# RishWijewardhena/vision-textile-inspection

Hardware: AMD Instinct MI355X
Metric: frames/sec whole-node, YOLOv8n-seg 640x640 bs=64; mask IoU vs CPU ref (higher is better)
Workload: dtype f16x2

## Files before the change

vision-textile-inspection_amd/csrc/post.hip:

```cpp
#include <algorithm>
#include <cmath>
#include <cstdio>
#include <cstring>
#include <type_traits>
#include <vector>

#include "vti_internal.h"

namespace vti {

typedef _Float16 half_t;
typedef _Float16 half8 __attribute__((ext_vector_type(8)));
typedef float f32x4 __attribute__((ext_vector_type(4)));

struct LinTap { int s0, s1, a0, a1; };

__device__ __forceinline__ LinTap lin_tap(int d, int ssize, double scale, bool horizontal) {
    float f = (float)(((double)d + 0.5) * scale - 0.5);
    int s = (int)floorf(f);
    f -= (float)s;
    LinTap t;
    if (horizontal) {
        if (s < 0) { s = 0; f = 0.f; }
        if (s >= ssize - 1) { s = ssize - 1; f = 0.f; }
// ... 89 lines not shown
                    const int rr = i / (ncol * 3), j = i - rr * ncol * 3;
                    band[((size_t)rr * W + xb) * 3 + j] = s_px[rr][j];
                }
            }
        }
        return;
    }
    const bool src4 = ((uintptr_t)src & 3) == 0, out4 = ((uintptr_t)out & 3) == 0;
    const bool wide = src4 && (copy ? ((W0 | left) & 3) == 0 : (left & 1) == 0);
    for (int g = tid; g < (W >> 2); g += 256) {
        const int dx0 = 4 * g - left;
        const bool inside = dx0 >= 0 && dx0 + 3 < new_w;
        uint8_t* o = band + (size_t)g * 12;
        for (int rr = 0; rr < rows; ++rr, o += (size_t)W * 3) {
            const int dy = y0 + rr - top;
            unsigned w[3] = {0x72727272u, 0x72727272u, 0x72727272u};
            if (dy >= 0 && dy < new_h && dx0 + 3 >= 0 && dx0 < new_w) {
                if (copy) {
                    const uint8_t* s = src + ((long long)dy * W0 + dx0) * 3;
                    if (wide && inside) {
                        const unsigned* q = (const unsigned*)s;
                        w[0] = q[0]; w[1] = q[1]; w[2] = q[2];
                    } else {
#pragma unroll
                        for (int i = 0; i < 12; ++i) {
                            const int dx = dx0 + i / 3;
                            const unsigned v = dx >= 0 && dx < new_w ? s[i] : 114u;
                            w[i >> 2] = (w[i >> 2] & ~(255u << ((i & 3) * 8))) | (v << ((i & 3) * 8));
                        }
                    }
                } else {
                    const uint8_t* s0 = src + ((long long)(2 * dy) * W0 + 2 * dx0) * 3;
                    const uint8_t* s1 = s0 + (size_t)W0 * 3;
                    if (wide && inside) {
                        unsigned q0[6], q1[6];
#pragma unroll
                        for (int i = 0; i < 6; ++i) { q0[i] = ((const unsigned*)s0)[i]; q1[i] = ((const unsigned*)s1)[i]; }
#pragma unroll
                        for (int i = 0; i < 12; ++i) {
                            const int j = 6 * (i / 3) + i % 3;
                            const unsigned v = (lb_byte(q0, j) + lb_byte(q0, j + 3) + lb_byte(q1, j) + lb_byte(q1, j + 3) + 2) >> 2;
                            w[i >> 2] = (w[i >> 2] & ~(255u << ((i & 3) * 8))) | (v << ((i & 3) * 8));
                        }
                    } else {
#pragma unroll
                        for (int i = 0; i < 12; ++i) {
                            const int dx = dx0 + i / 3, j = 6 * (i / 3) + i % 3;
                            unsigned v = 114u;
                            if (dx >= 0 && dx < new_w) v = (s0[j] + s0[j + 3] + s1[j] + s1[j + 3] + 2) >> 2;
                            w[i >> 2] = (w[i >> 2] & ~(255u << ((i & 3) * 8))) | (v << ((i & 3) * 8));
                        }
                    }
                }
            }
            if (out4) {
                *(uint3*)o = make_uint3(w[0], w[1], w[2]);
            } else {
#pragma unroll
                for (int i = 0; i < 12; ++i) o[i] = (uint8_t)lb_byte(w, i);
            }
        }
    }
}

hipError_t launch_letterbox(const uint8_t* frames, int B, int H0, int W0, const FrameRow* table, uint8_t* out, int H, int W,
                            hipStream_t st) {
    if (B == 0) return hipSuccess;
    if (W & 3) return hipErrorInvalidValue;
    const dim3 grid((H + LB_ROWS - 1) / LB_ROWS, B);
    FrameRow one = {};
    if (table) hipLaunchKernelGGL(letterbox_rows_kernel<true>, grid, dim3(256), 0, st, frames, one, table, out, H, W);
    else {
        frame_row_fill(H, W, H0, W0, 0, one);
        hipLaunchKernelGGL(letterbox_rows_kernel<false>, grid, dim3(256), 0, st, frames, one, table, out, H, W);
    }
    return hipGetLastError();
}

constexpr int NMS_THREADS = 1024;
constexpr int NMS_LDS_BOX = 2048;
constexpr int NMS_LDS_KEYS = 2048;
constexpr float NMS_MAX_WH = 7680.0f;
constexpr int NMS_MAX_NMS = 30000;

static inline size_t nms_pow2(size_t n) { size_t p = 1; while (p < n) p <<= 1; return p; }
static inline size_t align256(size_t n) { return (n + 255) & ~(size_t)255; }

struct NmsWsLayout { size_t keys, keys2, boxes, area, cls, keep, kid, kcls, per_frame; };
static NmsWsLayout nms_layout(int A) {
    NmsWsLayout l;
    size_t off = 0;
    l.keys = off; off += align256(nms_pow2((size_t)A) * 8);
    l.keys2 = off; off += align256(nms_pow2((size_t)A) * 8);
    l.boxes = off; off += align256((size_t)A * 16);
    l.area = off; off += align256((size_t)A * 4);
    l.cls = off; off += align256((size_t)A * 4);
    l.keep = off; off += align256((size_t)A * 4);
    l.kid = off; off += align256((size_t)A * 4);
    l.kcls = off; off += align256((size_t)A * 4);
    l.per_frame = off;
    return l;
}
size_t nms_workspace_bytes(int B, int A) { return nms_layout(A).per_frame * (size_t)B + align256((size_t)B * 4) + align256((size_t)B * A * 8); }
float* nms_workspace_best(void* ws, int B, int A) { return (float*)((char*)ws + nms_layout(A).per_frame * (size_t)B + align256((size_t)B * 4)); }

__global__ __launch_bounds__(256) void nms_scan_kernel(const float* __restrict__ pred, int A, int nc, int nm, float conf,
                                                       char* ws, NmsWsLayout L, int* __restrict__ ncand, float* __restrict__ best_out) {
    const int b = blockIdx.y;
    const int no = 4 + nc + nm;
    float best;
    int j = 0;
    int a;
    if (((no | nc) & 3) == 0) {
        a = blockIdx.x * 64 + (threadIdx.x >> 2);
        const int q = threadIdx.x & 3;
        best = -INFINITY; j = 0x7fffffff;
        if (a < A) {
            const float4* row = (const float4*)(pred + ((size_t)b * A + a) * no + 4);
            constexpr int MAXV = 8;
            float4 v[MAXV];
#pragma unroll
            for (int u = 0; u < MAXV; ++u) {
                const int i = q + 4 * u;
                v[u] = row[i < (nc >> 2) ? i : 0];
            }
#pragma unroll
            for (int u = 0; u < MAXV; ++u) {
                const int i = q + 4 * u;
                if (i >= (nc >> 2)) continue;
                if (v[u].x > best) { best = v[u].x; j = 4 * i; }
                if (v[u].y > best) { best = v[u].y; j = 4 * i + 1; }
                if (v[u].z > best) { best = v[u].z; j = 4 * i + 2; }
                if (v[u].w > best) { best = v[u].w; j = 4 * i + 3; }
            }
            for (int i = q + 4 * MAXV; i < (nc >> 2); i += 4) {
                const float4 w = row[i];
                if (w.x > best) { best = w.x; j = 4 * i; }
                if (w.y > best) { best = w.y; j = 4 * i + 1; }
                if (w.z > best) { best = w.z; j = 4 * i + 2; }
                if (w.w > best) { best = w.w; j = 4 * i + 3; }
            }
        }
#pragma unroll
        for (int o = 1; o <= 2; o <<= 1) {
            const float ob = __shfl_xor(best, o);
            const int oj = __shfl_xor(j, o);
            if (ob > best || (ob == best && oj < j)) { best = ob; j = oj; }
        }
        if (q != 0 || a >= A) return;
    } else {
        a = blockIdx.x * 256 + threadIdx.x;
        if (a >= A) return;
        const float* P = pred + ((size_t)b * A + a) * no;
        best = P[4];
        for (int c = 1; c < nc; ++c) {
            const float v = P[4 + c];
            if (v > best) { best = v; j = c; }
        }
    }
    if (best_out) {
        *(float2*)(best_out + ((size_t)b * A + a) * 2) = make_float2(best, (float)(j == 0x7fffffff ? 0 : j));
        return;
    }
    if (best > conf) {
        char* wsb = ws + (size_t)b * L.per_frame;
        const int idx = atomicAdd(&ncand[b], 1);
        ((unsigned long long*)(wsb + L.keys))[idx] = ((unsigned long long)(~__float_as_uint(best)) << 32) | (unsigned)a;
        ((int*)(wsb + L.cls))[a] = j;
    }
}

#ifdef VTI_STAMPS
__device__ unsigned long long g_nms_stamps[4096 * 8];
#define NMS_STAMP(i)                                                                                   \
    do {                                                                                               \
        if (tid == 0 && b < 4096) {                                                                    \
            unsigned long long t_;                                                                     \
            asm volatile("s_memtime %0\n\ts_waitcnt lgkmcnt(0)" : "=s"(t_)::"memory");                 \
            g_nms_stamps[b * 8 + (i)] = t_;                                                            \
        }                                                                                              \
    } while (0)
#else
#define NMS_STAMP(i) do { } while (0)
#endif

template <typename KeyP, typename BoxP, typename FltP, typename IntP>
__device__ __forceinline__ void nms_body(const float* __restrict__ P, int A, int nc, int nm, int n, double iou, int max_det,
                                         int agnostic, float* __restrict__ D, int* __restrict__ counts, int b,
                                         const unsigned long long* __restrict__ g_keys_in, KeyP keys, BoxP boxes, FltP area,
                                         IntP keep, IntP kid, IntP kcls, unsigned char* suppressed,
                                         const int* __restrict__ cls_of) {
    const int tid = threadIdx.x;
    int Pn = 1;
    while (Pn < n) Pn <<= 1;
    for (int i = tid; i < Pn; i += NMS_THREADS) keys[i] = i < n ? g_keys_in[i] : ~0ull;
    __syncthreads();
    for (int k = 2; k <= Pn; k <<= 1) {
        for (int j = k >> 1; j > 0; j >>= 1) {
            for (int i = tid; i < Pn; i += NMS_THREADS) {
                const int ixj = i ^ j;
                if (ixj > i) {
                    const unsigned long long x = keys[i], y = keys[ixj];
                    const bool up = (i & k) == 0;
                    if ((x > y) == up) { keys[i] = y; keys[ixj] = x; }
                }
            }
            __syncthreads();
        }
    }
    NMS_STAMP(1);
    if (n > NMS_MAX_NMS) n = NMS_MAX_NMS;
    for (int i = tid; i < n; i += NMS_THREADS) {
        const int a = (int)(keys[i] & 0xffffffffu);
        const float* Pa = P + (size_t)a * (4 + nc + nm);
        const float cx = Pa[0], cy = Pa[1], w = Pa[2], h = Pa[3];
        const float dw = w / 2.0f, dh = h / 2.0f;
        const float off = agnostic ? 0.0f : (float)cls_of[a] * NMS_MAX_WH;
        f32x4 bx;
        bx[0] = (cx - dw) + off; bx[1] = (cy - dh) + off; bx[2] = (cx + dw) + off; bx[3] = (cy + dh) + off;
        boxes[i] = bx;
        area[i] = (bx[2] - bx[0]) * (bx[3] - bx[1]);
        suppressed[i] = 0;
    }
    __syncthreads();
    NMS_STAMP(2);
    __shared__ unsigned long long s_rows[64];
    __shared__ int s_kept;
    auto iou_gt = [&](const f32x4& bi, float ai, const f32x4& bj, float aj) -> bool {
        const float xx1 = fmaxf(bi[0], bj[0]), yy1 = fmaxf(bi[1], bj[1]);
        const float xx2 = fminf(bi[2], bj[2]), yy2 = fminf(bi[3], bj[3]);
        const float w = fmaxf(0.0f, xx2 - xx1), h = fmaxf(0.0f, yy2 - yy1);
        const float inter = w * h;
        const float ovr = inter / (ai + aj - inter);
        return (double)ovr > iou;
    };
    int kept = 0;
    if (tid == 0) s_kept = 0;
    for (int base = 0; base < n && kept < max_det; base += 64) {
        const int cnt = min(64, n - base);
        if (tid < 64) s_rows[tid] = 0;
        __syncthreads();
        for (int e = tid; e < 64 * 16; e += NMS_THREADS) {
            const int i = e >> 4, jg = (e & 15) * 4;
            if (i >= cnt || jg + 3 <= i) continue;
            const f32x4 bi = boxes[base + i];
            const float ai = area[base + i];
            unsigned long long m = 0;
            f32x4 bj4[4];
            float aj4[4];
#pragma unroll
            for (int k = 0; k < 4; ++k) {
                const int jc = jg + k < cnt ? jg + k : cnt - 1;
                bj4[k] = boxes[base + jc]; aj4[k] = area[base + jc];
            }
#pragma unroll
            for (int k = 0; k < 4; ++k) {
                const int j = jg + k;
                if (j > i && j < cnt && iou_gt(bi, ai, bj4[k], aj4[k])) m |= 1ull << j;
            }
            if (m) atomicOr(&s_rows[i], m);
        }
        __syncthreads();
        if (tid < 64) {
            const bool alive_l = tid < cnt && !suppressed[base + tid];
            unsigned long long alive = __ballot(alive_l);
            int k_ = kept;
            const unsigned long long myrow = s_rows[tid];
            const int row_lo = (int)(unsigned)myrow, row_hi = (int)(unsigned)(myrow >> 32);
            while (alive && k_ < max_det) {
                const int i = __ffsll((long long)alive) - 1;
                if (tid == 0) keep[k_] = base + i;
                ++k_;
                const unsigned long long ri = (unsigned long long)(unsigned)__builtin_amdgcn_readlane(row_lo, i) |
                                              ((unsigned long long)(unsigned)__builtin_amdgcn_readlane(row_hi, i) << 32);
                alive &= ~(ri | (1ull << i));
            }
            if (tid == 0) s_kept = k_;
        }
        __syncthreads();
        const int kept0 = kept;
        kept = s_kept;
        if (kept < max_det) {
            const int nk = kept - kept0;
            const int rest = n - (base + 64);
            int parts = 1;
            while (parts < 8 && rest * parts * 2 <= NMS_THREADS) parts <<= 1;
            const int part = tid & (parts - 1), lane_j = tid / parts, jstep = NMS_THREADS / parts;
            for (int j = base + 64 + lane_j; j < n; j += jstep) {
                if (suppressed[j]) continue;
                const f32x4 bj = boxes[j];
                const float aj = area[j];
                bool sup = false;
                for (int t = 4 * part; t < nk && !sup; t += 4 * parts) {
                    int ii[4];
                    f32x4 bk[4];
                    float ak[4];
#pragma unroll
                    for (int u = 0; u < 4; ++u) ii[u] = keep[kept0 + (t + u < nk ? t + u : nk - 1)];
#pragma unroll
                    for (int u = 0; u < 4; ++u) { bk[u] = boxes[ii[u]]; ak[u] = area[ii[u]]; }
#pragma unroll
                    for (int u = 0; u < 4; ++u) sup = sup | iou_gt(bk[u], ak[u], bj, aj);
                }
                if (sup) suppressed[j] = 1;
            }
        }
        __syncthreads();
    }
    NMS_STAMP(3);
    for (int k = tid; k < kept; k += NMS_THREADS) {
        const int a = (int)(keys[keep[k]] & 0xffffffffu);
        kid[k] = a;
        kcls[k] = cls_of[a];
    }
    __syncthreads();
    const int row = 6 + nm;
    const unsigned row_magic = (unsigned)((0x100000000ull + (unsigned)row - 1) / (unsigned)row);
    const int nel = kept * row, ntot = max_det * row;
    const int no_ = 4 + nc + nm;
    constexpr int OU = 8;
    for (int e0 = tid; e0 < nel; e0 += OU * NMS_THREADS) {
        float x1[OU], x2[OU];
        int fj[OU];
#pragma unroll
        for (int u = 0; u < OU; ++u) {
            const int e = e0 + u * NMS_THREADS;
            const int ec = e < nel ? e : 0;
            const int k = (int)__umulhi((unsigned)ec, row_magic), f = ec - k * row;
            const int a = kid[k], j = kcls[k];
            const int off1 = f < 4 ? (f & 1) : f == 4 ? 4 + j : f == 5 ? 0 : 4 + nc + (f - 6);
            const int off2 = f < 4 ? 2 + (f & 1) : off1;
            const float* Pa = P + (size_t)a * no_;
            x1[u] = Pa[off1]; x2[u] = Pa[off2];
            fj[u] = (f << 16) | j;
        }
#pragma unroll
        for (int u = 0; u < OU; ++u) {
            const int e = e0 + u * NMS_THREADS;
            const int f = fj[u] >> 16, j = fj[u] & 0xffff;
            const float d_ = x2[u] / 2.0f;
            const float v = f < 2 ? x1[u] - d_ : f < 4 ? x1[u] + d_ : f == 5 ? (float)j : x1[u];
            if (e < nel) D[e] = v;
        }
    }
    for (int e = nel + tid; e < ntot; e += NMS_THREADS) D[e] = 0.f;
    __syncthreads();
    NMS_STAMP(4);
    if (tid == 0) counts[b] = kept;
}

__global__ __launch_bounds__(NMS_THREADS) void nms_kernel(const float* __restrict__ pred, int A, int nc, int nm,
                                                          float conf, double iou, int max_det, int agnostic,
                                                          float* __restrict__ dets, int* __restrict__ counts,
                                                          char* ws, NmsWsLayout L, int* __restrict__ ncand,
                                                          const float* __restrict__ best) {
    extern __shared__ __attribute__((aligned(16))) char smem[];
    unsigned long long* lds_keys = (unsigned long long*)smem;
    f32x4* lds_boxes = (f32x4*)(smem + NMS_LDS_KEYS * 8);
    float* lds_area = (float*)(lds_boxes + NMS_LDS_BOX);
    int* lds_keep = (int*)(lds_area + NMS_LDS_BOX);
    unsigned char* suppressed = (unsigned char*)(lds_keep + 3 * NMS_LDS_BOX);

    const int b = blockIdx.x, tid = threadIdx.x;
    const int no = 4 + nc + nm;
    const float* P = pred + (size_t)b * no * A;
    char* wsb = ws + (size_t)b * L.per_frame;
    unsigned long long* g_keys = (unsigned long long*)(wsb + L.keys);
    const int* cls_of = (const int*)(wsb + L.cls);
    float* D = dets + (size_t)b * max_det * (6 + nm);
    __shared__ int s_cnt;
    if (best) {
        if (tid == 0) s_cnt = 0;
        __syncthreads();
        const float2* bp = (const float2*)best + (size_t)b * A;
        int* cls_w = (int*)(wsb + L.cls);
        for (int a0 = 0; a0 < A; a0 += 4 * NMS_THREADS) {
            float2 v[4];
#pragma unroll
            for (int u = 0; u < 4; ++u) { const int a = a0 + tid + u * NMS_THREADS; v[u] = bp[a < A ? a : A - 1]; }
#pragma unroll
            for (int u = 0; u < 4; ++u) {
                const int a = a0 + tid + u * NMS_THREADS;
                if (a < A && v[u].x > conf) {
                    const int idx = atomicAdd(&s_cnt, 1);
                    g_keys[idx] = ((unsigned long long)(~__float_as_uint(v[u].x)) << 32) | (unsigned)a;
                    cls_w[a] = (int)v[u].y;
                }
            }
        }
        __syncthreads();
        if (tid == 0) ncand[b] = s_cnt;
    }
    const int n = best ? s_cnt : ncand[b];
    if (n == 0) {
        if (tid == 0) counts[b] = 0;
        for (int i = tid; i < max_det * (6 + nm); i += NMS_THREADS) D[i] = 0.f;
        return;
    }
    NMS_STAMP(0);
    if (n <= NMS_LDS_BOX && max_det <= NMS_LDS_BOX) {
        nms_body(P, A, nc, nm, n, iou, max_det, agnostic, D, counts, b, g_keys, lds_keys, lds_boxes, lds_area, lds_keep,
                 lds_keep + NMS_LDS_BOX, lds_keep + 2 * NMS_LDS_BOX, suppressed, cls_of);
    } else {
        int* g_int = (int*)(wsb + L.keep);
        nms_body(P, A, nc, nm, n, iou, max_det, agnostic, D, counts, b, g_keys, (unsigned long long*)(wsb + L.keys2),
                 (f32x4*)(wsb + L.boxes), (float*)(wsb + L.area), g_int, (int*)(wsb + L.kid), (int*)(wsb + L.kcls), suppressed,
                 cls_of);
    }
}

hipError_t launch_anchor_best(const float* pred, int B, int A, int nc, int nm, float* best, hipStream_t st) {
    if (B == 0) return hipSuccess;
    const int apb = (((4 + nc + nm) | nc) & 3) == 0 ? 64 : 256;
    hipLaunchKernelGGL(nms_scan_kernel, dim3((A + apb - 1) / apb, B), dim3(256), 0, st, pred, A, nc, nm, 0.0f, (char*)nullptr, nms_layout(A),
                       (int*)nullptr, best);
    return hipGetLastError();
}

hipError_t launch_nms(const float* pred, const float* best, int B, int A, int nc, int nm, float conf, double iou, int max_det,
                      int agnostic, float* dets, int* counts, void* ws, hipStream_t st) {
    if (B == 0) return hipSuccess;
    const size_t lds = (size_t)NMS_LDS_KEYS * 8 + (size_t)NMS_LDS_BOX * 32 + (((size_t)A + 15) & ~(size_t)15);
    if (lds > 150 * 1024) return hipErrorInvalidValue;
    const NmsWsLayout L = nms_layout(A);
    int* ncand = (int*)((char*)ws + L.per_frame * (size_t)B);
    if (!best) {
        hipError_t e = hipMemsetAsync(ncand, 0, sizeof(int) * (size_t)B, st);
        if (e != hipSuccess) return e;
        const int apb = (((4 + nc + nm) | nc) & 3) == 0 ? 64 : 256;
        hipLaunchKernelGGL(nms_scan_kernel, dim3((A + apb - 1) / apb, B), dim3(256), 0, st, pred, A, nc, nm, conf, (char*)ws, L, ncand, (float*)nullptr);
    }
    const hipError_t e = launch_lds<nms_kernel>(dim3(B), dim3(NMS_THREADS), lds, st, pred, A, nc, nm, conf, iou, max_det, agnostic,
                                                dets, counts, (char*)ws, L, ncand, best);
#ifdef VTI_STAMPS
    {
        (void)hipStreamSynchronize(st);
        static int calls = 0;
        if (++calls == 3) {
            std::vector<unsigned long long> h(4096 * 8);
            std::vector<int> hc(B), hn(B);
            (void)hipMemcpyFromSymbol(h.data(), HIP_SYMBOL(g_nms_stamps), h.size() * 8);
            (void)hipMemcpy(hc.data(), counts, B * 4, hipMemcpyDeviceToHost);
            (void)hipMemcpy(hn.data(), ncand, B * 4, hipMemcpyDeviceToHost);
            const char* nm_[4] = {"sort", "boxes", "greedy", "output"};
            int worst = 0;
            for (int b = 1; b < B; ++b) if (h[b * 8 + 4] - h[b * 8] > h[worst * 8 + 4] - h[worst * 8]) worst = b;
            fprintf(stderr, "[nms stamps] slowest frame %d: candidates %d kept %d\n", worst, hn[worst], hc[worst]);
            for (int i = 0; i < 4; ++i) {
                std::vector<long long> d;
                for (int b = 0; b < B; ++b) if (hn[b] > 0) d.push_back((long long)(h[b * 8 + i + 1] - h[b * 8 + i]));
                std::sort(d.begin(), d.end());
                fprintf(stderr, "[nms stamps] %-7s median %8lld  max %8lld  slowest-frame %8lld cycles\n", nm_[i],
                        d.empty() ? 0 : d[d.size() / 2], d.empty() ? 0 : d.back(), (long long)(h[worst * 8 + i + 1] - h[worst * 8 + i]));
            }
        }
    }
#endif
    return e;
}

constexpr int MT = 64;
constexpr int ML = MT / 4 + 3;

__global__ __launch_bounds__(256) void mask_offsets_kernel(const int* __restrict__ counts, int B, int max_det,
                                                           int* __restrict__ offsets, int* __restrict__ nitems) {
    extern __shared__ int s_off[];
    for (int b = threadIdx.x; b < B; b += 256) {
        int c = counts[b];
        s_off[b + 1] = c < 0 ? 0 : (c > max_det ? max_det : c);
    }
    if (threadIdx.x == 0) { s_off[0] = 0; *nitems = 0; }
    __syncthreads();
    if (threadIdx.x == 0)
        for (int b = 0; b < B; ++b) s_off[b + 1] += s_off[b];
    __syncthreads();
    for (int b = threadIdx.x; b <= B; b += 256) offsets[b] = s_off[b];
}

__device__ __forceinline__ void mask_slot_owner(const int* __restrict__ offsets, int B, int slot, int& b, int& inst) {
    int lo = 0, hi = B;
    while (hi - lo > 1) { const int mid = (lo + hi) >> 1; if (offsets[mid] <= slot) lo = mid; else hi = mid; }
    b = lo; inst = slot - offsets[lo];
}
__device__ __forceinline__ bool mask_tile_rect(const float* __restrict__ d, int H, int W, int& tx0, int& tx1, int& ty0, int& ty1) {
    const int tiles_x = (W + MT - 1) / MT, tiles_y = (H + MT - 1) / MT;
    const float x1 = d[0] - 8.f, y1 = d[1] - 8.f, x2 = d[2] + 8.f, y2 = d[3] + 8.f;
    tx0 = (int)floorf(x1 / MT); tx1 = (int)floorf(x2 / MT); ty0 = (int)floorf(y1 / MT); ty1 = (int)floorf(y2 / MT);
    tx0 = max(tx0, 0); ty0 = max(ty0, 0); tx1 = min(tx1, tiles_x - 1); ty1 = min(ty1, tiles_y - 1);
    return tx1 >= tx0 && ty1 >= ty0;
}

template <bool FUSED_OFFSETS>
__global__ __launch_bounds__(256) void mask_clear_kernel(const int* __restrict__ counts, int* __restrict__ offsets, int* __restrict__ nitems,
                                                         int B, int max_det, int slot_bytes, int capacity, uint8_t* __restrict__ masks) {
    const int slot = blockIdx.x;
    int total;
    if constexpr (FUSED_OFFSETS) {
        __shared__ int s_c[1025];
        __shared__ int s_tot;
        if (threadIdx.x == 0) s_tot = 0;
        __syncthreads();
        int part = 0;
        for (int b = threadIdx.x; b < B; b += 256) {
            const int c = counts[b], cc = c < 0 ? 0 : (c > max_det ? max_det : c);
            part += cc;
            if (slot == 0) s_c[b + 1] = cc;
        }
        for (int o = 32; o > 0; o >>= 1) part += __shfl_xor(part, o);
        if ((threadIdx.x & 63) == 0) atomicAdd(&s_tot, part);
        __syncthreads();
        total = s_tot;
        if (slot == 0) {
            if (threadIdx.x == 0) {
                s_c[0] = 0; *nitems = 0;
                for (int b = 0; b < B; ++b) s_c[b + 1] += s_c[b];
            }
// ... 141 lines not shown

        const float thr = mode == VTI_MASK_SIGMOID ? 0.5f : 0.0f;
        const int wv = tid >> 6, ln = tid & 63;
        const int yw = __builtin_amdgcn_readfirstlane(y0 + 16 * wv);
        if (yw >= H) continue;
        const int xg = x0 + ln;
        int k0 = xg >= 2 ? (xg - 2) >> 2 : 0;
        k0 = k0 < Wp - 1 ? k0 : Wp - 1;
        const int k1 = k0 + (k0 < Wp - 1 ? 1 : 0);
        const float lx1 = xg >= 2 ? 0.125f + 0.25f * (float)((xg - 2) & 3) : 0.0f;
        const int rb = (yw >> 2) - 1;
        int ro[6];
#pragma unroll
        for (int j = 0; j < 6; ++j) {
            int rr = rb + j;
            rr = rr < 0 ? 0 : (rr > Hp - 1 ? Hp - 1 : rr);
            ro[j] = (rr - ly0) * (ML + 1);
        }
        const int valid = W - x0;
        const unsigned long long cmask = valid >= 64 ? ~0ull : ((1ull << valid) - 1ull);
        unsigned lo = 0u, hi = 0u;
        if (packing == VTI_PACK_U8) mask_rows16<true>(&low[0][0], ro, k0 - lx0, k1 - lx0, lx1, yw == 0, thr, lo, hi, masks + (size_t)slot * H * W, W, H, yw, xg);
        else mask_rows16<false>(&low[0][0], ro, k0 - lx0, k1 - lx0, lx1, yw == 0, thr, lo, hi, nullptr, W, H, yw, xg);
        lo &= (unsigned)cmask; hi &= (unsigned)(cmask >> 32);
        if (packing != VTI_PACK_U8 && ln < 16 && yw + ln < H) {
            const int wb = W >> 3;
            unsigned* o = (unsigned*)(masks + ((size_t)slot * H + yw + ln) * wb + (x0 >> 3));
            o[0] = lo;
            if (valid >= 64) o[1] = hi;
        }
    }
}

constexpr int MLP = ML + 2;
__device__ __forceinline__ void mask_tile_rows64(const float* lrow, float wy, bool first, float thr, unsigned& lo, unsigned& hi) {
    float vv[18];
#pragma unroll
    for (int j = 0; j < 18; ++j) {
        const float a = lrow[j], b = lrow[j + MLP];
        vv[j] = __builtin_fmaf(b - a, wy, a);
    }
    unsigned w[2] = {0u, 0u};
    if (thr == 0.0f) {
#pragma unroll
        for (int j = 0; j < 18; ++j) vv[j] = -vv[j];
#pragma unroll
        for (int hf = 0; hf < 2; ++hf) {
#pragma unroll
            for (int k = 31; k >= 0; --k) {
                const int px = 32 * hf + k;
                const int jj = ((px - 2) >> 2) + 1;
                const float wx = 0.125f + 0.25f * (float)((px + 2) & 3);
                float u = __builtin_fmaf(vv[jj + 1] - vv[jj], wx, vv[jj]);
                if (px < 2) u = first ? vv[1] + 0.0f : u;
                w[hf] = __builtin_amdgcn_alignbit(w[hf], __builtin_bit_cast(unsigned, u), 31);
            }
        }
    } else {
#pragma unroll
        for (int hf = 0; hf < 2; ++hf) {
#pragma unroll
            for (int k = 31; k >= 0; --k) {
                const int px = 32 * hf + k;
                const int jj = ((px - 2) >> 2) + 1;
                const float wx = 0.125f + 0.25f * (float)((px + 2) & 3);
                float v = __builtin_fmaf(vv[jj + 1] - vv[jj], wx, vv[jj]);
                if (px < 2) v = first ? vv[1] : v;
                asm("v_cmp_gt_f32 vcc, %1, %2\n\tv_addc_co_u32 %0, vcc, %0, %0, vcc" : "+v"(w[hf]) : "v"(v), "v"(thr) : "vcc");
            }
        }
    }
    lo = w[0]; hi = w[1];
}

#ifdef VTI_STAMPS
__device__ unsigned long long g_mask_acc[8];
#define MASK_T(i) do { unsigned long long t_; asm volatile("s_memtime %0\n\ts_waitcnt lgkmcnt(0)" : "=s"(t_)::"memory"); \
                       macc[i] += t_ - mprev; mprev = t_; } while (0)
#else
#define MASK_T(i) do { } while (0)
#endif

constexpr int MG = 16;
constexpr int MPTS = ML * ML;
constexpr int MTILES = (MPTS + 15) / 16;
constexpr int MJ = (MTILES + 3) / 4;
constexpr int MROUND = 64;

template <bool F16>
__device__ __forceinline__ float mask_coef_operands(const float (&cf)[32], uint4* dst) {
    float scale = 1.0f;
    if constexpr (F16) {
        float mx = 0.f;
#pragma unroll
        for (int k = 0; k < 32; ++k) mx = fmaxf(mx, fabsf(cf[k]));
        float inv = 1.0f;
        if (!(mx < 3.0e4f)) {
            const int e = (int)((__builtin_bit_cast(unsigned, mx) >> 23) & 255u) - 127 - 13;
            const int ec = e < -100 ? -100 : (e > 100 ? 100 : e);
            scale = __builtin_bit_cast(float, (unsigned)(ec + 127) << 23);
            inv = __builtin_bit_cast(float, (unsigned)(127 - ec) << 23);
        }
#pragma unroll
        for (int q = 0; q < 4; ++q) {
            half8 hh, hl;
#pragma unroll
            for (int k = 0; k < 8; ++k) {
                const float c = cf[8 * q + k] * inv;
                const half_t h = (half_t)c;
                hh[k] = h;
                hl[k] = (half_t)(c - (float)h);
            }
            dst[q] = __builtin_bit_cast(uint4, hh);
            dst[4 + q] = __builtin_bit_cast(uint4, hl);
        }
    } else {
#pragma unroll
        for (int q = 0; q < 8; ++q)
            dst[q] = __builtin_bit_cast(uint4, (f32x4){cf[4 * q], cf[4 * q + 1], cf[4 * q + 2], cf[4 * q + 3]});
    }
    return scale;
}

template <typename T>
__global__ __launch_bounds__(256, sizeof(T) == 2 ? 4 : 3) void masks_group_kernel(const float* __restrict__ dets, const int* __restrict__ offsets,
                                                          const T* __restrict__ proto, int B, int max_det, int Hp, int Wp,
                                                          int H, int W, int mode, int packing, uint8_t* __restrict__ masks,
                                                          int capacity) {
    constexpr bool F16 = sizeof(T) == 2;
    constexpr int ROW = 6 + 32;
    typedef typename std::conditional<F16, half8, f32x4>::type opv;
    constexpr int NOP = F16 ? 1 : 2;
    __shared__ uint4 s_co[MROUND][8];
    __shared__ float4 s_box[MROUND];
    __shared__ float s_scale[MROUND];
    __shared__ unsigned short s_list[MROUND];
    __shared__ int s_n;
    __shared__ float low[MG][ML][MLP];
    const int tid = threadIdx.x, ln = tid & 63, wv = tid >> 6;
    const int li = ln & 15, lg = ln >> 4;
    const int tiles_x = (W + MT - 1) / MT, tiles_y = (H + MT - 1) / MT, tiles = tiles_x * tiles_y;
    const int n = B * tiles;
    const int nx = (int)gridDim.x >> 3, xcd = (int)blockIdx.x & 7, jx = (int)blockIdx.x >> 3;
    const int per = (n + 7) >> 3;
    const int it1 = min(n, (xcd + 1) * per);
    const float wr = (float)((double)Wp / (double)W), hr = (float)((double)Hp / (double)H);
    const float sh = (float)Hp / (float)H, sw = (float)Wp / (float)W;
    const float thr = mode == VTI_MASK_SIGMOID ? 0.5f : 0.0f;
    int prc[MJ];
#pragma unroll
    for (int j = 0; j < MJ; ++j) {
        const int m = wv + 4 * j, pt = 16 * m + li;
        const bool live = m < MTILES && pt < MPTS;
        const int r = live ? pt / ML : ML - 1, c = live ? pt - r * ML : ML;
        prc[j] = (r << 5) | c;
    }
#ifdef VTI_STAMPS
    unsigned long long macc[6] = {0, 0, 0, 0, 0, 0}, mprev, mitems = 0, mpairs = 0;
    asm volatile("s_memtime %0\n\ts_waitcnt lgkmcnt(0)" : "=s"(mprev)::"memory");
#endif
    for (int it = xcd * per + jx; it < it1; it += nx) {
        const int b = it / tiles, t = it - b * tiles;
        const int ty = t / tiles_x, tx = t - ty * tiles_x;
        const int y0 = ty * MT, x0 = tx * MT;
        const int off_b = offsets[b];
        const int n_b = min(offsets[b + 1], capacity) - off_b;
        if (n_b <= 0) continue;
        float fy0 = sh * ((float)y0 + 0.5f) - 0.5f; fy0 = fy0 < 0.f ? 0.f : fy0;
        float fx0 = sw * ((float)x0 + 0.5f) - 0.5f; fx0 = fx0 < 0.f ? 0.f : fx0;
        const int ly0 = (int)fy0, lx0 = (int)fx0;
        opv pb[MJ][NOP];
#pragma unroll
        for (int j = 0; j < MJ; ++j) {
            int q = prc[j];
            asm volatile("" : "+v"(q));
            const int py = ly0 + (q >> 5), px = lx0 + (q & 31);
            const int pyc = py < Hp ? py : Hp - 1, pxc = px < Wp ? px : Wp - 1;
            const T* pp = proto + ((size_t)(b * Hp + pyc) * Wp + pxc) * 32;
            if constexpr (F16) pb[j][0] = *(const half8*)(pp + 8 * lg);
            else { pb[j][0] = *(const f32x4*)(pp + 4 * lg); pb[j][1] = *(const f32x4*)(pp + 16 + 4 * lg); }
        }
        MASK_T(0);
        const int wvy = __builtin_amdgcn_readfirstlane(y0 + 16 * wv);
        const int xg = x0 + ln;
        int kc0 = xg >= 2 ? (xg - 2) >> 2 : 0;
        kc0 = kc0 < Wp - 1 ? kc0 : Wp - 1;
        const int kc1 = kc0 + (kc0 < Wp - 1 ? 1 : 0) - lx0;
        kc0 -= lx0;
        const float lx1 = xg >= 2 ? 0.125f + 0.25f * (float)((xg - 2) & 3) : 0.0f;
        const int rbase = (wvy >> 2) - 1;
        int ro[6];
#pragma unroll
        for (int j = 0; j < 6; ++j) {
            int rr = rbase + j;
            rr = rr < 0 ? 0 : (rr > Hp - 1 ? Hp - 1 : rr);
            ro[j] = (rr - ly0) * MLP;
        }
        const int valid = W - x0;
        const unsigned long long cmask = valid >= 64 ? ~0ull : ((1ull << valid) - 1ull);
        const int yr = y0 + ln;
        const int lrow_off = ((yr >= 2 ? (yr - 2) >> 2 : 0) - ly0) * MLP + (tx > 0 ? 0 : -1);
        const float wy = yr >= 2 ? 0.125f + 0.25f * (float)((yr - 2) & 3) : 0.0f;
        for (int i0 = 0; i0 < n_b; i0 += MROUND) {
            __syncthreads();
            if (wv == 0) {
                const int i = i0 + ln;
                const float* d = dets + ((size_t)b * max_det + (i < n_b ? i : n_b - 1)) * ROW;
                float2 raw[ROW / 2];
#pragma unroll
                for (int k = 0; k < ROW / 2; ++k) raw[k] = *(const float2*)(d + 2 * k);
                const float dd[4] = {raw[0].x, raw[0].y, raw[1].x, raw[1].y};
                int tx0, tx1, ty0, ty1;
                const bool hit = i < n_b && mask_tile_rect(dd, H, W, tx0, tx1, ty0, ty1) && tx >= tx0 && tx <= tx1 && ty >= ty0 && ty <= ty1;
                const unsigned long long bal = __builtin_amdgcn_ballot_w64(hit);
                if (ln == 0) s_n = __builtin_popcountll(bal);
                if (hit) {
                    const int pos = __builtin_amdgcn_mbcnt_hi((unsigned)(bal >> 32), __builtin_amdgcn_mbcnt_lo((unsigned)bal, 0u));
                    s_list[pos] = (unsigned short)ln;
                    s_box[pos] = make_float4(dd[0] * wr, dd[1] * hr, dd[2] * wr, dd[3] * hr);
                    float cf[32];
#pragma unroll
                    for (int k = 0; k < 16; ++k) { cf[2 * k] = raw[3 + k].x; cf[2 * k + 1] = raw[3 + k].y; }
                    s_scale[pos] = mask_coef_operands<F16>(cf, s_co[pos]);
                }
            }
            __syncthreads();
            const int nlist = s_n;
            MASK_T(1);
#ifdef VTI_STAMPS
            ++mitems; mpairs += nlist;
#endif
            for (int g0 = 0; g0 < nlist; g0 += MG) {
                const int ng = min(MG, nlist - g0);
                opv ca[2];
                ca[0] = __builtin_bit_cast(opv, s_co[g0 + li][lg]);
                ca[1] = __builtin_bit_cast(opv, s_co[g0 + li][4 + lg]);
                float4 rb[4];
                float rs[4];
#pragma unroll
                for (int r = 0; r < 4; ++r) {
                    const int u = 4 * lg + r;
                    rb[r] = s_box[g0 + u];
                    rs[r] = s_scale[g0 + u];
                }
#pragma unroll
                for (int j = 0; j < MJ; ++j) {
                    f32x4 acc = (f32x4){0.f, 0.f, 0.f, 0.f};
                    if constexpr (F16) {
                        acc = __builtin_amdgcn_mfma_f32_16x16x32_f16(ca[0], pb[j][0], acc, 0, 0, 0);
                        acc = __builtin_amdgcn_mfma_f32_16x16x32_f16(ca[1], pb[j][0], acc, 0, 0, 0);
                    } else {
#pragma unroll
                        for (int q = 0; q < 2; ++q)
#pragma unroll
                            for (int k = 0; k < 4; ++k) acc = __builtin_amdgcn_mfma_f32_16x16x4f32(ca[q][k], pb[j][q][k], acc, 0, 0, 0);
                    }
                    float v[4];
#pragma unroll
                    for (int r = 0; r < 4; ++r) v[r] = F16 ? acc[r] * rs[r] : acc[r];
                    if (mode == VTI_MASK_SIGMOID) {
#pragma unroll
                        for (int r = 0; r < 4; ++r) v[r] = 1.0f / (1.0f + expf(-v[r]));
                    }
                    int q = prc[j];
                    asm volatile("" : "+v"(q));
                    const int pr = q >> 5, pc = q & 31, py = min(ly0 + pr, Hp - 1), px = min(lx0 + pc, Wp - 1);
                    const float pfc = (float)px, pfr = (float)py;
                    const int pla = pr * MLP + pc;
#pragma unroll
                    for (int r = 0; r < 4; ++r) {
                        const bool inb = pfc >= rb[r].x && pfc < rb[r].z && pfr >= rb[r].y && pfr < rb[r].w;
                        (&low[4 * lg + r][0][0])[pla] = (inb && v[r] == v[r]) ? v[r] : 0.f;
                    }
                }
                MASK_T(2);
                __syncthreads();
                MASK_T(3);
                if (packing != VTI_PACK_U8) {
                    for (int u = wv; u < ng; u += 4) {
                        const int slot = off_b + i0 + (int)s_list[g0 + u];
                        unsigned lo, hi;
                        mask_tile_rows64(&low[u][0][0] + lrow_off, wy, tx == 0, thr, lo, hi);
                        lo &= (unsigned)cmask; hi &= (unsigned)(cmask >> 32);
                        if (yr < H) {
                            unsigned* o = (unsigned*)(masks + ((size_t)slot * H + yr) * (W >> 3) + (x0 >> 3));
                            if (valid >= 64 && !(W & 63)) *(uint2*)o = make_uint2(lo, hi);
                            else {
                                o[0] = lo;
                                if (valid >= 64) o[1] = hi;
                            }
                        }
                    }
                } else if (wvy < H) {
                    for (int u = 0; u < ng; ++u) {
                        const int slot = off_b + i0 + (int)s_list[g0 + u];
                        unsigned lo = 0u, hi = 0u;
                        mask_rows16<true>(&low[u][0][0], ro, kc0, kc1, lx1, wvy == 0, thr, lo, hi, masks + (size_t)slot * H * W, W, H, wvy, xg);
                    }
                }
                MASK_T(4);
                if (g0 + MG < nlist) __syncthreads();
                MASK_T(5);
            }
        }
    }
#ifdef VTI_STAMPS
    if (tid == 0) {
        for (int i = 0; i < 6; ++i) atomicAdd(&g_mask_acc[i], macc[i]);
        atomicAdd(&g_mask_acc[6], mitems); atomicAdd(&g_mask_acc[7], mpairs);
    }
#endif
}

size_t masks_workspace_bytes(int capacity, int H, int W) {
    const size_t tiles = (size_t)((H + MT - 1) / MT) * ((W + MT - 1) / MT);
    return 256 + ((((size_t)capacity * tiles * 8) + 255) & ~(size_t)255);
}

hipError_t launch_masks(int dtype, const float* dets, const int* counts, const void* proto, int B, int max_det, int nm,
                        int Hp, int Wp, int H, int W, int mode, int packing, uint8_t* masks, int capacity,
                        int* offsets, void* ws, hipStream_t st) {
    if (B == 0) return hipSuccess;
    if (Hp * 4 != H || Wp * 4 != W || nm > 64) return hipErrorInvalidValue;
    int* nitems = (int*)ws;
    int2* items = (int2*)((char*)ws + 256);
    if (max_det > 65535 || B > 32767 || H > 64 * MT || W > 64 * MT || capacity > (1 << 19)) return hipErrorInvalidValue;
    const size_t slot_bytes = (size_t)H * (packing == VTI_PACK_U8 ? W : W / 8);
    if (capacity > 0 && ((slot_bytes & 15) || ((uintptr_t)masks & 15))) return hipErrorInvalidValue;
    if (capacity > 0 && B <= 1024) {
        hipLaunchKernelGGL(mask_clear_kernel<true>, dim3(capacity), dim3(256), 0, st, counts, offsets, nitems, B, max_det, (int)slot_bytes, capacity, masks);
    } else {
        hipLaunchKernelGGL(mask_offsets_kernel, dim3(1), dim3(256), (size_t)(B + 1) * sizeof(int), st, counts, B, max_det, offsets, nitems);
        if (capacity <= 0) return hipGetLastError();
        hipLaunchKernelGGL(mask_clear_kernel<false>, dim3(capacity), dim3(256), 0, st, counts, offsets, nitems, B, max_det, (int)slot_bytes, capacity, masks);
    }
    const int per_cu = dtype == VTI_F16 ? (nm == 32 ? resident_per_cu<masks_group_kernel<half_t>>(256, 4, 8) : resident_per_cu<masks_kernel<half_t>>(256, 4, 8))
                                        : (nm == 32 ? resident_per_cu<masks_group_kernel<float>>(256, 4, 8) : resident_per_cu<masks_kernel<float>>(256, 4, 8));
    int grid = 256 * per_cu;
    if (const char* e = getenv("VTI_MASK_WGS_PER_CU")) grid = 256 * std::max(1, std::min(per_cu, atoi(e)));
    if (nm == 32) {
        if (dtype == VTI_F16)
            hipLaunchKernelGGL(masks_group_kernel<half_t>, dim3(grid), dim3(256), 0, st, dets, offsets, (const half_t*)proto, B, max_det, Hp, Wp,
                               H, W, mode, packing, masks, capacity);
        else
            hipLaunchKernelGGL(masks_group_kernel<float>, dim3(grid), dim3(256), 0, st, dets, offsets, (const float*)proto, B, max_det, Hp, Wp,
                               H, W, mode, packing, masks, capacity);
#ifdef VTI_STAMPS
        {
            (void)hipStreamSynchronize(st);
            static int calls = 0;
            if (++calls == 3) {
                unsigned long long h[8];
                (void)hipMemcpyFromSymbol(h, HIP_SYMBOL(g_mask_acc), sizeof h);
                const char* nm_[6] = {"decode + issue protos", "list build", "coeffs + MFMA + low", "barrier", "upsample + store", "barrier (next group)"};
                fprintf(stderr, "[mask stamps] %llu (frame, tile) items, %llu (instance, tile) pairs over %d calls (wave 0 of each block; s_memtime ticks per item)\n", h[6], h[7], calls);
                for (int i = 0; i < 6; ++i) fprintf(stderr, "[mask stamps] %-22s %9.1f\n", nm_[i], (double)h[i] / (double)h[6]);
            }
        }
#endif
        return hipGetLastError();
    }
    hipLaunchKernelGGL(mask_plan_kernel, dim3((capacity + 255) / 256), dim3(256), 0, st, dets, offsets, B, max_det, 6 + nm, H, W,
                       capacity, items, nitems);
    if (dtype == VTI_F16)
        hipLaunchKernelGGL(masks_kernel<half_t>, dim3(grid), dim3(256), 0, st, dets, offsets, (const half_t*)proto, B, max_det, nm, Hp, Wp,
                           H, W, mode, packing, masks, items, nitems);
    else
        hipLaunchKernelGGL(masks_kernel<float>, dim3(grid), dim3(256), 0, st, dets, offsets, (const float*)proto, B, max_det, nm, Hp, Wp,
                           H, W, mode, packing, masks, items, nitems);
    return hipGetLastError();
}

int native_mask_layout(int Hp, int Wp, int H0, int W0, int packing, int out[6]) {
    if (Hp < 1 || Wp < 1 || H0 < 1 || W0 < 1 || (packing != VTI_PACK_U8 && packing != VTI_PACK_BITS)) return -1;
    const double mh = Hp, mw = Wp;
    const double gain = std::min(mh / H0, mw / W0);
    const double pad_w = (mw - W0 * gain) / 2, pad_h = (mh - H0 * gain) / 2;
    const int top = (int)pad_h, left = (int)pad_w, bottom = (int)(mh - pad_h), right = (int)(mw - pad_w);
    if (top < 0 || left < 0 || bottom <= top || right <= left || bottom > Hp || right > Wp) return -1;
    const long long row_bytes = packing == VTI_PACK_BITS ? 8LL * ((W0 + 63) / 64) : (long long)W0;
    const long long slot_bytes = row_bytes * H0;
    if (slot_bytes > 0x7fffffffLL) return -1;
    out[0] = top; out[1] = bottom; out[2] = left; out[3] = right; out[4] = (int)row_bytes; out[5] = (int)slot_bytes;
    return 0;
}

constexpr int NTW = 64;
constexpr int NPTS = 512;
constexpr int NJ = NPTS / 16 / 4;

struct NativeMaskParams {
    const float* dets;
    const float* xyxy;
    const int* offsets;
    const void* proto;
    uint8_t* masks;
    size_t slot_bytes;
    int B, max_det, Hp, Wp, H0, W0;
    int top, left, inH, inW;
    float sy, sx;
    int th;
    int row_contig, col_contig;
    int mode, packing, row_bytes, capacity;
};

__device__ __forceinline__ void native_tap(int d, float s, int in, int& i0, int& i1, float& lam) {
    float src = s * ((float)d + 0.5f) - 0.5f;
    src = src < 0.f ? 0.f : src;
    i0 = (int)src;
    i0 = i0 < in - 1 ? i0 : in - 1;
    i1 = i0 + (i0 < in - 1 ? 1 : 0);
    lam = src - (float)i0;
}
__device__ __forceinline__ int native_src(int f, int d0, int contig, int base, float s, int in) {
    if (contig) return base + f;
    int i0, i1;
    float lam;
    native_tap(d0 + (f >> 1), s, in, i0, i1, lam);
    return (f & 1) ? i1 : i0;
}
__device__ __forceinline__ void native_span(int d0, int n, int contig, float s, int in, int& base, int& len) {
    if (!contig) { base = 0; len = 2 * n; return; }
    int a0, a1, b0, b1;
    float lam;
    native_tap(d0, s, in, a0, a1, lam);
// ... 369 lines not shown
```

Measured before the change: 15420.

## Add full IoU bitmask NMS path and split-f16 MFMA mask path for fp32 protos

NMS gains a path for frames with at most 512 candidates. It builds the full pairwise IoU suppression bitmask in LDS with wave ballots, then resolves the greedy keep list in a single wave, replacing the block-by-block loop with its per-block barriers. Separately, fp32 prototypes in the f16x2 (VTI_H2) dtype now run a split hi/lo half-precision MFMA path: prototypes are rescaled and split into two halves and combined over three f16 MFMAs instead of the fp32 MFMA sequence. The split path trades exactness for tensor-core throughput, and it encodes NaN results as a large negative value, which changes how masks are thresholded.

Result: no change. 15320 (-0.6%).

```diff
diff --git a/vision-textile-inspection_amd/csrc/post.hip b/vision-textile-inspection_amd/csrc/post.hip
--- a/vision-textile-inspection_amd/csrc/post.hip
+++ b/vision-textile-inspection_amd/csrc/post.hip
@@ -195,6 +195,8 @@
 constexpr int NMS_LDS_KEYS = 2048;
 constexpr float NMS_MAX_WH = 7680.0f;
 constexpr int NMS_MAX_NMS = 30000;
+constexpr int NMS_MAT_N = 512;
+constexpr int NMS_MAT_W = NMS_MAT_N / 64;
 
 static inline size_t nms_pow2(size_t n) { size_t p = 1; while (p < n) p <<= 1; return p; }
 static inline size_t align256(size_t n) { return (n + 255) & ~(size_t)255; }
@@ -302,7 +304,7 @@
                                          int agnostic, float* __restrict__ D, int* __restrict__ counts, int b,
                                          const unsigned long long* __restrict__ g_keys_in, KeyP keys, BoxP boxes, FltP area,
                                          IntP keep, IntP kid, IntP kcls, unsigned char* suppressed,
-                                         const int* __restrict__ cls_of) {
+                                         unsigned long long* mat, bool mat_ok, const int* __restrict__ cls_of) {
     const int tid = threadIdx.x;
     int Pn = 1;
     while (Pn < n) Pn <<= 1;
@@ -349,7 +351,65 @@
     };
     int kept = 0;
     if (tid == 0) s_kept = 0;
-    for (int base = 0; base < n && kept < max_det; base += 64) {
+    const bool full_matrix = mat_ok && n <= NMS_MAT_N;
+    if (full_matrix) {
+        const int nw = (n + 63) >> 6;
+        const int ln = tid & 63;
+        for (int u = __builtin_amdgcn_readfirstlane(tid >> 6); u < 2 * nw * (nw + 1); u += NMS_THREADS / 64) {
+            int w = 0;
+            while (2 * (w + 1) * (w + 2) <= u) ++w;
+            const int i0 = 16 * (u - 2 * w * (w + 1));
+            const int j = 64 * w + ln, jc = j < n ? j : n - 1;
+            const f32x4 bj = boxes[jc];
+            const float aj = area[jc];
+            const int i1 = min(i0 + 16, n);
+            for (int i = i0; i < i1; ++i) {
+                const unsigned long long m = __ballot(j > i && j < n && iou_gt(boxes[i], area[i], bj, aj));
+                if (ln == 0) mat[i * NMS_MAT_W + w] = m;
+            }
+        }
+        __syncthreads();
+        if (tid < 64) {
+            unsigned long long removed = 0;
+            const int w8 = tid & 7, part = tid >> 3;
+            int k_ = 0;
+            for (int blk = 0; blk < nw && k_ < max_det; ++blk) {
+                const int base = 64 * blk, cnt = min(64, n - base);
+                const unsigned long long myrow = tid < cnt ? mat[(base + tid) * NMS_MAT_W + blk] : 0ull;
+                const int row_lo = (int)(unsigned)myrow, row_hi = (int)(unsigned)(myrow >> 32);
+                const unsigned long long rem = (unsigned long long)(unsigned)__builtin_amdgcn_readlane((int)(unsigned)removed, blk) |
+                                               ((unsigned long long)(unsigned)__builtin_amdgcn_readlane((int)(unsigned)(removed >> 32), blk) << 32);
+                unsigned long long alive = (cnt == 64 ? ~0ull : (1ull << cnt) - 1ull) & ~rem;
+                unsigned long long kept_m = 0;
+                while (alive && k_ < max_det) {
+                    const int i = __ffsll((long long)alive) - 1;
+                    if (tid == 0) keep[k_] = base + i;
+                    ++k_;
+                    kept_m |= 1ull << i;
+                    const unsigned long long ri = (unsigned long long)(unsigned)__builtin_amdgcn_readlane(row_lo, i) |
+                                                  ((unsigned long long)(unsigned)__builtin_amdgcn_readlane(row_hi, i) << 32);
+                    alive &= ~(ri | (1ull << i));
+                }
+                if (blk + 1 < nw && k_ < max_det) {
+                    unsigned long long acc = 0;
+#pragma unroll
+                    for (int q = 0; q < 8; ++q) {
+                        const int r = part + 8 * q;
+                        const unsigned long long v = mat[(base + r) * NMS_MAT_W + w8];
+                        acc |= ((kept_m >> r) & 1ull) && w8 > blk && w8 < nw ? v : 0ull;
+                    }
+                    acc |= __shfl_xor(acc, 8);
+                    acc |= __shfl_xor(acc, 16);
+                    acc |= __shfl_xor(acc, 32);
+                    removed |= acc;
+                }
+            }
+            if (tid == 0) s_kept = k_;
+        }
+        __syncthreads();
+        kept = s_kept;
+    }
+    for (int base = 0; !full_matrix && base < n && kept < max_det; base += 64) {
         const int cnt = min(64, n - base);
         if (tid < 64) s_rows[tid] = 0;
         __syncthreads();
@@ -466,13 +526,14 @@
                                                           float conf, double iou, int max_det, int agnostic,
                                                           float* __restrict__ dets, int* __restrict__ counts,
                                                           char* ws, NmsWsLayout L, int* __restrict__ ncand,
-                                                          const float* __restrict__ best) {
+                                                          const float* __restrict__ best, int use_mat) {
     extern __shared__ __attribute__((aligned(16))) char smem[];
     unsigned long long* lds_keys = (unsigned long long*)smem;
     f32x4* lds_boxes = (f32x4*)(smem + NMS_LDS_KEYS * 8);
     float* lds_area = (float*)(lds_boxes + NMS_LDS_BOX);
     int* lds_keep = (int*)(lds_area + NMS_LDS_BOX);
     unsigned char* suppressed = (unsigned char*)(lds_keep + 3 * NMS_LDS_BOX);
+    unsigned long long* lds_mat = (unsigned long long*)(suppressed + ((A + 15) & ~15));
 
     const int b = blockIdx.x, tid = threadIdx.x;
     const int no = 4 + nc + nm;
@@ -513,12 +574,12 @@
     NMS_STAMP(0);
     if (n <= NMS_LDS_BOX && max_det <= NMS_LDS_BOX) {
         nms_body(P, A, nc, nm, n, iou, max_det, agnostic, D, counts, b, g_keys, lds_keys, lds_boxes, lds_area, lds_keep,
-                 lds_keep + NMS_LDS_BOX, lds_keep + 2 * NMS_LDS_BOX, suppressed, cls_of);
+                 lds_keep + NMS_LDS_BOX, lds_keep + 2 * NMS_LDS_BOX, suppressed, lds_mat, use_mat != 0, cls_of);
     } else {
         int* g_int = (int*)(wsb + L.keep);
         nms_body(P, A, nc, nm, n, iou, max_det, agnostic, D, counts, b, g_keys, (unsigned long long*)(wsb + L.keys2),
                  (f32x4*)(wsb + L.boxes), (float*)(wsb + L.area), g_int, (int*)(wsb + L.kid), (int*)(wsb + L.kcls), suppressed,
-                 cls_of);
+                 lds_mat, false, cls_of);
     }
 }
 
@@ -533,8 +594,11 @@
 hipError_t launch_nms(const float* pred, const float* best, int B, int A, int nc, int nm, float conf, double iou, int max_det,
                       int agnostic, float* dets, int* counts, void* ws, hipStream_t st) {
     if (B == 0) return hipSuccess;
-    const size_t lds = (size_t)NMS_LDS_KEYS * 8 + (size_t)NMS_LDS_BOX * 32 + (((size_t)A + 15) & ~(size_t)15);
+    size_t lds = (size_t)NMS_LDS_KEYS * 8 + (size_t)NMS_LDS_BOX * 32 + (((size_t)A + 15) & ~(size_t)15);
     if (lds > 150 * 1024) return hipErrorInvalidValue;
+    const size_t mat_bytes = (size_t)NMS_MAT_N * NMS_MAT_W * 8;
+    const int use_mat = lds + mat_bytes <= 150 * 1024;
+    if (use_mat) lds += mat_bytes;
     const NmsWsLayout L = nms_layout(A);
     int* ncand = (int*)((char*)ws + L.per_frame * (size_t)B);
     if (!best) {
@@ -544,7 +608,7 @@
         hipLaunchKernelGGL(nms_scan_kernel, dim3((A + apb - 1) / apb, B), dim3(256), 0, st, pred, A, nc, nm, conf, (char*)ws, L, ncand, (float*)nullptr);
     }
     const hipError_t e = launch_lds<nms_kernel>(dim3(B), dim3(NMS_THREADS), lds, st, pred, A, nc, nm, conf, iou, max_det, agnostic,
-                                                dets, counts, (char*)ws, L, ncand, best);
+                                                dets, counts, (char*)ws, L, ncand, best, use_mat);
 #ifdef VTI_STAMPS
     {
         (void)hipStreamSynchronize(st);
@@ -852,12 +916,13 @@
 #endif
 
 constexpr int MG = 16;
+constexpr float MASK_NAN_LOW = -0x1p126f;
 constexpr int MPTS = ML * ML;
 constexpr int MTILES = (MPTS + 15) / 16;
 constexpr int MJ = (MTILES + 3) / 4;
 constexpr int MROUND = 64;
 
-template <bool F16>
+template <bool F16, bool SPLITK = false>
 __device__ __forceinline__ float mask_coef_operands(const float (&cf)[32], uint4* dst) {
     float scale = 1.0f;
     if constexpr (F16) {
@@ -876,7 +941,7 @@
             half8 hh, hl;
 #pragma unroll
             for (int k = 0; k < 8; ++k) {
-                const float c = cf[8 * q + k] * inv;
+                const float c = cf[SPLITK ? 4 * q + (k & 3) + 4 * (k & 4) : 8 * q + k] * inv;
                 const half_t h = (half_t)c;
                 hh[k] = h;
                 hl[k] = (half_t)(c - (float)h);
@@ -892,14 +957,17 @@
     return scale;
 }
 
-template <typename T>
+template <typename T, bool SPLIT = false>
 __global__ __launch_bounds__(256, sizeof(T) == 2 ? 4 : 3) void masks_group_kernel(const float* __restrict__ dets, const int* __restrict__ offsets,
                                                           const T* __restrict__ proto, int B, int max_det, int Hp, int Wp,
                                                           int H, int W, int mode, int packing, uint8_t* __restrict__ masks,
                                                           int capacity) {
+    static_assert(!SPLIT || sizeof(T) == 4, "SPLIT is the fp32-prototype path");
     constexpr bool F16 = sizeof(T) == 2;
+    constexpr bool C16 = F16 || SPLIT;
     constexpr int ROW = 6 + 32;
     typedef typename std::conditional<F16, half8, f32x4>::type opv;
+    typedef typename std::conditional<C16, half8, f32x4>::type copv;
     constexpr int NOP = F16 ? 1 : 2;
     __shared__ uint4 s_co[MROUND][8];
     __shared__ float4 s_box[MROUND];
@@ -940,6 +1008,9 @@
         float fx0 = sw * ((float)x0 + 0.5f) - 0.5f; fx0 = fx0 < 0.f ? 0.f : fx0;
         const int ly0 = (int)fy0, lx0 = (int)fx0;
         opv pb[MJ][NOP];
+        float ps[MJ];
+#pragma unroll
+        for (int j = 0; j < MJ; ++j) ps[j] = 1.0f;
 #pragma unroll
         for (int j = 0; j < MJ; ++j) {
             int q = prc[j];
@@ -991,20 +1062,52 @@
                     float cf[32];
 #pragma unroll
                     for (int k = 0; k < 16; ++k) { cf[2 * k] = raw[3 + k].x; cf[2 * k + 1] = raw[3 + k].y; }
-                    s_scale[pos] = mask_coef_operands<F16>(cf, s_co[pos]);
+                    s_scale[pos] = mask_coef_operands<C16, SPLIT>(cf, s_co[pos]);
                 }
             }
             __syncthreads();
             const int nlist = s_n;
             MASK_T(1);
+            if constexpr (SPLIT) {
+                if (i0 == 0) {
+#pragma unroll
+                    for (int j = 0; j < MJ; ++j) {
+                        float p[8];
+#pragma unroll
+                        for (int k = 0; k < 8; ++k) p[k] = pb[j][k >> 2][k & 3];
+                        float mx = 0.f;
+#pragma unroll
+                        for (int k = 0; k < 8; ++k) mx = fmaxf(mx, fabsf(p[k]));
+                        mx = fmaxf(mx, __shfl_xor(mx, 16));
+                        mx = fmaxf(mx, __shfl_xor(mx, 32));
+                        float inv = 1.0f;
+                        if (mx > 0.f) {
+                            const int e = (int)((__builtin_bit_cast(unsigned, mx) >> 23) & 255u) - 127 - 13;
+                            const int ec = e < -126 ? -126 : (e > 126 ? 126 : e);
+                            ps[j] = __builtin_bit_cast(float, (unsigned)(ec + 127) << 23);
+                            inv = __builtin_bit_cast(float, (unsigned)(127 - ec) << 23);
+                        }
+                        half8 hh, hl;
+#pragma unroll
+                        for (int k = 0; k < 8; ++k) {
+                            const float c = p[k] * inv;
+                            const half_t h = (half_t)c;
+                            hh[k] = h;
+                            hl[k] = (half_t)(c - (float)h);
+                        }
+                        pb[j][0] = __builtin_bit_cast(f32x4, hh);
+                        pb[j][1] = __builtin_bit_cast(f32x4, hl);
+                    }
+                }
+            }
 #ifdef VTI_STAMPS
             ++mitems; mpairs += nlist;
 #endif
             for (int g0 = 0; g0 < nlist; g0 += MG) {
                 const int ng = min(MG, nlist - g0);
-                opv ca[2];
-                ca[0] = __builtin_bit_cast(opv, s_co[g0 + li][lg]);
-                ca[1] = __builtin_bit_cast(opv, s_co[g0 + li][4 + lg]);
+                copv ca[2];
+                ca[0] = __builtin_bit_cast(copv, s_co[g0 + li][lg]);
+                ca[1] = __builtin_bit_cast(copv, s_co[g0 + li][4 + lg]);
                 float4 rb[4];
                 float rs[4];
 #pragma unroll
@@ -1019,6 +1122,11 @@
                     if constexpr (F16) {
                         acc = __builtin_amdgcn_mfma_f32_16x16x32_f16(ca[0], pb[j][0], acc, 0, 0, 0);
                         acc = __builtin_amdgcn_mfma_f32_16x16x32_f16(ca[1], pb[j][0], acc, 0, 0, 0);
+                    } else if constexpr (SPLIT) {
+                        const half8 ph = __builtin_bit_cast(half8, pb[j][0]), pl = __builtin_bit_cast(half8, pb[j][1]);
+                        acc = __builtin_amdgcn_mfma_f32_16x16x32_f16(ca[1], ph, acc, 0, 0, 0);
+                        acc = __builtin_amdgcn_mfma_f32_16x16x32_f16(ca[0], pl, acc, 0, 0, 0);
+                        acc = __builtin_amdgcn_mfma_f32_16x16x32_f16(ca[0], ph, acc, 0, 0, 0);
                     } else {
 #pragma unroll
                         for (int q = 0; q < 2; ++q)
@@ -1027,7 +1135,7 @@
                     }
                     float v[4];
 #pragma unroll
-                    for (int r = 0; r < 4; ++r) v[r] = F16 ? acc[r] * rs[r] : acc[r];
+                    for (int r = 0; r < 4; ++r) v[r] = SPLIT ? acc[r] * rs[r] * ps[j] : F16 ? acc[r] * rs[r] : acc[r];
                     if (mode == VTI_MASK_SIGMOID) {
 #pragma unroll
                         for (int r = 0; r < 4; ++r) v[r] = 1.0f / (1.0f + expf(-v[r]));
@@ -1040,7 +1148,7 @@
 #pragma unroll
                     for (int r = 0; r < 4; ++r) {
                         const bool inb = pfc >= rb[r].x && pfc < rb[r].z && pfr >= rb[r].y && pfr < rb[r].w;
-                        (&low[4 * lg + r][0][0])[pla] = (inb && v[r] == v[r]) ? v[r] : 0.f;
+                        (&low[4 * lg + r][0][0])[pla] = v[r] == v[r] ? (inb ? v[r] : 0.f) : (SPLIT ? MASK_NAN_LOW : 0.f);
                     }
                 }
                 MASK_T(2);
@@ -1105,12 +1213,17 @@
         hipLaunchKernelGGL(mask_clear_kernel<false>, dim3(capacity), dim3(256), 0, st, counts, offsets, nitems, B, max_det, (int)slot_bytes, capacity, masks);
     }
     const int per_cu = dtype == VTI_F16 ? (nm == 32 ? resident_per_cu<masks_group_kernel<half_t>>(256, 4, 8) : resident_per_cu<masks_kernel<half_t>>(256, 4, 8))
-                                        : (nm == 32 ? resident_per_cu<masks_group_kernel<float>>(256, 4, 8) : resident_per_cu<masks_kernel<float>>(256, 4, 8));
+                  : nm != 32        ? resident_per_cu<masks_kernel<float>>(256, 4, 8)
+                  : dtype == VTI_H2 ? resident_per_cu<masks_group_kernel<float, true>>(256, 4, 8)
+                                    : resident_per_cu<masks_group_kernel<float>>(256, 4, 8);
     int grid = 256 * per_cu;
     if (const char* e = getenv("VTI_MASK_WGS_PER_CU")) grid = 256 * std::max(1, std::min(per_cu, atoi(e)));
     if (nm == 32) {
         if (dtype == VTI_F16)
             hipLaunchKernelGGL(masks_group_kernel<half_t>, dim3(grid), dim3(256), 0, st, dets, offsets, (const half_t*)proto, B, max_det, Hp, Wp,
+                               H, W, mode, packing, masks, capacity);
+        else if (dtype == VTI_H2)
+            hipLaunchKernelGGL((masks_group_kernel<float, true>), dim3(grid), dim3(256), 0, st, dets, offsets, (const float*)proto, B, max_det, Hp, Wp,
                                H, W, mode, packing, masks, capacity);
         else
             hipLaunchKernelGGL(masks_group_kernel<float>, dim3(grid), dim3(256), 0, st, dets, offsets, (const float*)proto, B, max_det, Hp, Wp,
```
